# juanmc2005/diart

Hardware: AMD Instinct MI355X
Metric: real-time-factor xRT streams/GPU @500ms step (higher is better)
Workload: dtype f16x3

## Files before the change

### diart_amd/_lib.py

```python
from __future__ import annotations

import ctypes as C
import os
from pathlib import Path
from typing import Optional

EXPERIMENTS = os.environ.get("DZ_EXPERIMENTS", "0") not in ("", "0")
_LIB_PATH = Path(__file__).resolve().parent / ("libdiart_amd_exp.so" if EXPERIMENTS else "libdiart_amd.so")
_lib: Optional[C.CDLL] = None

c_float_p = C.POINTER(C.c_float)
c_double_p = C.POINTER(C.c_double)
c_int_p = C.POINTER(C.c_int)
vp = C.c_void_p


class SincNetWeights(C.Structure):
    _fields_ = [("wav_gamma", C.c_float), ("wav_beta", C.c_float)] + [
        (n, vp) for n in ("filt", "in0_g", "in0_b", "w1", "b1", "in1_g", "in1_b",
                          "w2", "b2", "in2_g", "in2_b", "w1_split", "w2_split", "filt_split")]


class SegWeights(C.Structure):
    _fields_ = [("sinc", SincNetWeights), ("wih", vp * 4), ("bih", vp * 4), ("whh", vp * 4),
# ... 89 lines not shown
    "dz_clu_step": (C.c_int, [vp, vp, C.c_int, C.c_int, vp, C.c_int, vp, vp]),
    "dz_clu_step_batch": (C.c_int, [C.POINTER(vp), C.c_int, vp, C.c_int, C.c_int, vp, C.c_int,
                                    vp, vp, C.c_int]),
    "dz_clu_get_centers": (C.c_int, [vp, vp, C.c_int]),
    "dz_clu_get_active": (C.c_int, [vp, vp]),
    "dz_clu_dim": (C.c_int, [vp]),
    "dz_clu_set_state": (C.c_int, [vp, vp, vp, C.c_int]),
    "dz_clu_destroy": (C.c_int, [vp]),
    "dz_lsap": (C.c_int, [vp, C.c_int, C.c_int, vp]),
    "dz_ring_create": (C.c_int, [vp, C.c_int, C.c_int, C.c_int, C.c_int, C.POINTER(vp)]),
    "dz_ring_reset": (C.c_int, [vp]),
    "dz_ring_destroy": (C.c_int, [vp]),
    "dz_ring_push": (C.c_int, [vp, vp, C.c_longlong, C.c_int, vp]),
    "dz_ring_window": (C.c_int, [vp, C.POINTER(vp), C.POINTER(C.c_longlong), C.POINTER(C.c_int)]),
    "dz_ring_read": (C.c_int, [vp, vp, vp]),
    "dz_ring_push_rows": (C.c_int, [vp, vp, C.c_longlong, C.c_int, C.POINTER(C.c_int), C.c_int, vp]),
    "dz_ring_filled_row": (C.c_int, [vp, C.c_int, C.POINTER(C.c_int)]),
    "dz_ring_gather": (C.c_int, [vp, C.POINTER(C.c_int), C.c_int, vp, C.c_longlong, vp]),
    "dz_ring_reset_row": (C.c_int, [vp, C.c_int]),
    "dz_tail_create": (C.c_int, [C.c_int, C.c_int, C.c_double, C.c_double, C.c_double, C.c_int,
                                 C.c_int, vp, C.POINTER(vp)]),
    "dz_tail_reset": (C.c_int, [vp]),
    "dz_tail_destroy": (C.c_int, [vp]),
    "dz_tail_max_rows": (C.c_int, [vp]),
    "dz_tail_step": (C.c_int, [vp, vp, C.c_double, C.c_double, vp, vp, vp, vp, vp, C.c_int, vp]),
    "dz_tail_step_batch": (C.c_int, [C.POINTER(vp), C.c_int, vp, vp, vp, vp, vp, vp, vp, vp,
                                     C.c_int, vp, C.c_int]),
    "dz_file_step_batch": (C.c_int, [C.POINTER(vp), C.POINTER(vp), C.c_int, vp, vp, vp, C.c_int, C.c_int, vp, C.c_int,
                                     C.c_int, vp, C.c_double, vp, C.c_int, vp, vp, C.c_int]),
    "dz_k_convgemm": (C.c_int, [vp, vp, vp]),
    "dz_k_gemm_f32": (C.c_int, [vp, vp, vp]),
    "dz_k_gemm_split": (C.c_int, [vp, vp, vp]),
    "dz_k_gemm_pre": (C.c_int, [vp, vp, vp]),
    "dz_k_mlp_head": (C.c_int, [vp, vp, C.c_longlong, vp, vp, vp, vp, vp, vp, C.c_int, C.c_int, C.c_int, C.c_int,
                                C.c_int, C.c_float, C.c_float, vp, vp, vp]),
    "dz_k_seg_head": (C.c_int, [vp, vp, vp, vp, C.c_int, C.c_int, C.c_int, C.c_int, C.c_int, vp, C.c_float,
                                C.c_float, C.c_int, vp, vp]),
    "dz_k_conv_pool": (C.c_int, [vp, vp, vp]),
    "dz_k_convgemm_ntile": (C.c_int, [C.c_int]),
    "dz_k_wave_stats": (C.c_int, [vp, vp, C.c_longlong, C.c_int, C.c_int, vp, vp]),
    "dz_k_sinc_conv0": (C.c_int, [vp, vp, C.c_longlong, C.c_int, C.c_int, vp, C.c_float,
                                  C.c_float, vp, vp, vp, vp]),
    "dz_k_sinc_conv0_split": (C.c_int, [vp, vp, C.c_longlong, C.c_int, C.c_int, vp, C.c_float,
                                        C.c_float, vp, vp, vp, vp]),
    "dz_k_conv0_split_ntile": (C.c_int, [C.c_int]),
    "dz_k_finalize_norm": (C.c_int, [vp, vp, C.c_int, C.c_int, C.c_int, C.c_int, vp, vp, vp, vp, vp]),
    "dz_k_lstm": (C.c_int, [vp, vp, vp, vp, C.c_int, C.c_int, vp]),
    "dz_k_lstm_mfma": (C.c_int, [vp, vp, vp, vp, C.c_int, C.c_int, C.c_int, C.c_int, vp]),
    "dz_k_lstm_planes": (C.c_int, [vp, vp, vp, vp, C.c_int, vp, C.c_longlong, C.c_int, C.c_int, vp]),
    "dz_k_stats_pool": (C.c_int, [vp, vp, C.c_int, C.c_int, C.c_int, vp, C.c_int, C.c_int,
                                  C.c_int, vp, C.c_int, vp]),
    "dz_k_powerset": (C.c_int, [vp, vp, C.c_int, C.c_int, C.c_int, vp, vp]),
}


EXPERIMENT_SIGNATURES = {
    "dz_k_gemm_g2": (C.c_int, [vp, vp, C.c_int, vp]),
    "dz_k_gemm_g3": (C.c_int, [vp, vp, C.c_int, vp]),
    "dz_k_conv_pool_debug": (C.c_int, [vp]),
    "dz_sinc_conv0_pair": (C.c_int, [vp, vp, vp, C.c_longlong, C.c_int, vp, vp, vp, vp]),
    "dz_k_sinc_conv0_pair": (C.c_int, [vp, vp, C.c_longlong, C.c_int, C.c_int, vp, vp, vp, C.c_float, C.c_float, vp, vp,
                                       vp, vp, vp]),
}


class ConvGemmDesc(C.Structure):
# ... 94 lines not shown
```

### diart_amd/csrc/api.hip

```cpp
#include "dz_common.h"

#include <stdarg.h>
#include <stdio.h>
#include <stdlib.h>
#include <string.h>
#include <mutex>
#include <new>

static thread_local char g_err[512] = "";
void dz_set_error(const char* fmt, ...) {
    va_list ap;
    va_start(ap, fmt);
    vsnprintf(g_err, sizeof(g_err), fmt, ap);
    va_end(ap);
}
extern "C" const char* dz_last_error(void) { return g_err; }
extern "C" int dz_version(void) { return DZ_VERSION; }
extern "C" int dz_abi_struct_sizes(int out[5]) {
    if (!out) return 2;
    out[0] = (int)sizeof(dz_sincnet_weights);
    out[1] = (int)sizeof(dz_seg_weights);
    out[2] = (int)sizeof(dz_emb_weights);
    out[3] = (int)sizeof(dz_ecapa_weights);
    out[4] = (int)sizeof(dz_convgemm_desc);
// ... 495 lines not shown
    const float* lin = nullptr;
    for (int layer = 0; layer < 4; ++layer) {
        DzConvGemm p;
        memset(&p, 0, sizeof(p));
        float* const gxl = layer == 0 ? s->gx0 : s->gx;
        p.W = s->w.wih[layer]; p.bias = s->w.bih[layer]; p.Y = gxl;
        p.taps = 1; p.dil = 1; p.Npad = 1024; p.Nstore = 1024; p.ldy = 1024; p.epi = DZ_EPI_BIAS;
        const bool do_proj = layer == 0 ? phase != 2 : phase != 1;
        const bool do_rec = phase != 1;
        if (layer == 0) {
            p.X = s->ss.y2;
            sinc_out_norm(p, s->w.sinc, s->g, s->ss, s->w.wih_split[0] != nullptr);
            p.B = B; p.Tin = p.Tout = p.Tstore = F; p.Cin = 64; p.K = 64; p.Kpad = 64; p.ldx = 64;
            p.xbs = (long long)F * 64; p.ybs = (long long)F * 1024;
        } else {
            p.X = lin;
            p.B = 1; p.Tin = p.Tout = p.Tstore = B * F; p.Cin = 256; p.K = 256; p.Kpad = 256;
            p.ldx = 256;
        }
        const bool pre0 = layer == 0 && s->pre && sinc_pre_split_ok(s->w.sinc, s->w.wih0_split_kb);
        if (layer == 0 && !pre0 && !s->w.wih_split[0] && sinc_f32_norm_pass(s->w.sinc)) {
            p.X = s->ss.y2s; p.norm_on_load = 0; p.npart = nullptr; p.nscale = p.nshift = nullptr;
            p.B = 1; p.Tin = p.Tout = p.Tstore = B * F; p.xbs = p.ybs = 0;
        }
        if (do_proj && pre0) {
            if ((rc = sinc_norm_split(s->w.sinc, s->g, s->ss, B, st))) return rc;
            p.X = nullptr; p.norm_on_load = 0; p.npart = nullptr; p.nscale = p.nshift = nullptr;
            p.B = 1; p.Tin = p.Tout = p.Tstore = B * F; p.xbs = p.ybs = 0;
        }
        if (do_proj)
        { ProfScope ps(layer == 0 ? T_PROJ0 : T_PROJ, B);
          if (pre0) {
              p.Xsplit = s->ss.y2s; p.xplane = rows * 64; p.Wsplit = s->w.wih0_split_kb;
              rc = dz_launch_gemm_pre(p, st);
          } else if (layer > 0 && s->pre) {
              p.X = nullptr; p.Xsplit = lin; p.xplane = rows * 256; p.Wsplit = s->w.wih_split[layer];
              rc = dz_launch_gemm_pre(p, st);
          } else {
              rc = run_gemm(p, s->w.wih_split[layer], st);
          }
          if (rc) return rc; }
        if (!do_rec) {
            s->front_B = B;
            return 0;
        }
        float* hout = (layer & 1) ? s->h1 : s->h0;
        { ProfScope ps(T_REC, B);
          float* hf = s->pre ? nullptr : hout;
          void* hs = s->pre ? (void*)hout : nullptr;
          rc = s->w.whh_split[layer]
                   ? dz_launch_lstm_mfma(gxl, s->w.whh_split[layer], hf, hs, rows * 256, B, F, 1,
                                         s->w.lstm_variant, st)
                   : dz_launch_lstm(gxl, s->w.whh[layer], hf, hs, rows * 256, B, F, 1, st);
          if (rc) return rc; }
        if (layer == 0) {
            DZ_HIP(hipEventRecord(s->ev_gx0_free, st));
            s->front_B = 0;
        }
        lin = hout;
    }
    DzConvGemm p;
    memset(&p, 0, sizeof(p));
    p.B = 1; p.Tin = p.Tout = p.Tstore = B * F; p.taps = 1; p.dil = 1;
    p.W = s->w.lin0_w; p.bias = s->w.lin0_b;
    p.Cin = 256; p.K = 256; p.Kpad = 256; p.ldx = 256; p.Npad = 128; p.Nstore = 128; p.ldy = 128;
    p.epi = DZ_EPI_BIAS_LEAKY;
    if (s->pre && mlp_head_enabled() && !(d_osp && normalize) && s->w.num_classes <= 8) {
        DzMlpHead m{};
        m.Xsplit = lin; m.xplane = rows * 256;
        m.W0split = s->w.lin0_split; m.W1split = s->w.lin1_split;
// ... 349 lines not shown
                               int n_streams, int k_local, int g_global, int dim, double* d_out,
                               void* stream) {
    DZ_REQUIRE(ctx && d_emb && d_centers && d_out, "dz_cdist_cosine: NULL argument");
    DZ_REQUIRE(n_streams >= 1 && k_local >= 1 && g_global >= 1 && dim >= 1,
               "dz_cdist_cosine: empty input");
    DZ_HIP(hipSetDevice(ctx->device));
    return dz_launch_cdist(d_emb, d_centers, n_streams, k_local, g_global, dim, d_out,
                           (hipStream_t)stream);
}

extern "C" int dz_k_convgemm(dz_ctx* ctx, const dz_convgemm_desc* d, void* stream) {
    DZ_REQUIRE(ctx && d, "dz_k_convgemm: NULL argument");
    DZ_HIP(hipSetDevice(ctx->device));
    DzRangeScope range_scope(ctx->oflag_dev);
    return dz_launch_convgemm(*d, (hipStream_t)stream);
}
extern "C" int dz_k_gemm_f32(dz_ctx* ctx, const dz_convgemm_desc* d, void* stream) {
    DZ_REQUIRE(ctx && d, "dz_k_gemm_f32: NULL argument");
    DZ_HIP(hipSetDevice(ctx->device));
    return dz_launch_gemm_f32(*d, (hipStream_t)stream);
}
extern "C" int dz_k_gemm_split(dz_ctx* ctx, const dz_convgemm_desc* d, void* stream) {
    DZ_REQUIRE(ctx && d, "dz_k_gemm_split: NULL argument");
    DZ_HIP(hipSetDevice(ctx->device));
    DzRangeScope range_scope(ctx->oflag_dev);
    return dz_launch_gemm_split(*d, (hipStream_t)stream);
}
extern "C" int dz_k_gemm_pre(dz_ctx* ctx, const dz_convgemm_desc* d, void* stream) {
    DZ_REQUIRE(ctx && d, "dz_k_gemm_pre: NULL argument");
    DZ_HIP(hipSetDevice(ctx->device));
    DzRangeScope range_scope(ctx->oflag_dev);
    return dz_launch_gemm_pre(*d, (hipStream_t)stream);
}
#ifdef DZ_EXPERIMENTS
extern "C" int dz_k_gemm_g2(dz_ctx* ctx, const dz_convgemm_desc* d, int row_fragments, void* stream) {
    DZ_REQUIRE(ctx && d, "dz_k_gemm_g2: NULL argument");
    DZ_REQUIRE(d->Wsplit && d->Xsplit && (d->Y || d->Ysplit) && d->B == 1 && d->K == d->Kpad && d->K == d->taps * d->Cin &&
                   d->Cin % 32 == 0 && d->Npad % 128 == 0 && d->pad == 0 && !d->X2 && !d->rowbias && d->ksplit <= 1 &&
                   !d->norm_on_load && d->Tout > 0 && d->Tout == d->Tin - (d->taps - 1) * d->dil && d->ldx % 32 == 0 &&
                   d->xplane % d->ldx == 0 && d->xplane / d->ldx >= d->Tin,
               "dz_k_gemm_g2: the requirements of dz_k_gemm_pre apply");
    DZ_HIP(hipSetDevice(ctx->device));
    DzRangeScope range_scope(ctx->oflag_dev);
    DzConvGemm p = *d;
    if (!p.oflag) p.oflag = ctx->oflag_dev;
    return dz_launch_gemm_g2(p, row_fragments, (hipStream_t)stream);
}
extern "C" int dz_k_gemm_g3(dz_ctx* ctx, const dz_convgemm_desc* d, int row_fragments, void* stream) {
    DZ_REQUIRE(ctx && d, "dz_k_gemm_g3: NULL argument");
    DZ_REQUIRE(d->Wsplit && d->Xsplit && (d->Y || d->Ysplit) && d->B == 1 && d->K == d->Kpad && d->K == d->taps * d->Cin &&
                   d->Cin % 32 == 0 && d->Npad % 128 == 0 && d->pad == 0 && !d->X2 && !d->rowbias && d->ksplit <= 1 &&
                   !d->norm_on_load && d->Tout > 0 && d->Tout == d->Tin - (d->taps - 1) * d->dil && d->ldx % 32 == 0 &&
                   d->xplane % d->ldx == 0 && d->xplane / d->ldx >= d->Tin,
               "dz_k_gemm_g3: the requirements of dz_k_gemm_pre apply");
    DZ_HIP(hipSetDevice(ctx->device));
    DzRangeScope range_scope(ctx->oflag_dev);
    DzConvGemm p = *d;
    if (!p.oflag) p.oflag = ctx->oflag_dev;
    return dz_launch_gemm_g3(p, row_fragments, (hipStream_t)stream);
}
#endif
extern "C" int dz_k_mlp_head(dz_ctx* ctx, const void* xsplit, long long xplane, const void* w0split,
                             const void* w1split, const float* b0, const float* b1, const float* cw,
                             const float* cb, int rows, int frames, int classes, int speakers, int powerset,
                             float gamma, float beta, float* d_seg, float* d_weights, void* stream) {
    DZ_REQUIRE(ctx, "dz_k_mlp_head: NULL argument");
// ... 161 lines not shown
```

### diart_amd/csrc/dz_common.h

```cpp
#pragma once
#include <hip/hip_runtime.h>
#include <hip/hip_ext.h>
#include <stdint.h>
#include <stddef.h>
#include <mutex>
#include "../../include/diart_amd.h"

#ifdef DZ_EXPERIMENTS
#include <stdlib.h>
static inline const char* dz_exp_env(const char* name) { return getenv(name); }
#else
#define dz_exp_env(name) ((const char*)nullptr)
#endif
enum { DZ_OPT_F32_GEMM = 0, DZ_OPT_POOL_FUSE, DZ_OPT_PACK_CACHE, DZ_OPT_COUNT };
int dz_option(int id);

typedef float f32x4 __attribute__((ext_vector_type(4)));
typedef float f32x2 __attribute__((ext_vector_type(2)));

#define DZ_MFMA(a, b, c) __builtin_amdgcn_mfma_f32_16x16x4f32((a), (b), (c), 0, 0, 0)

#define DZ_LEAKY_SLOPE 0.01f

struct DzAttrOnce {
// ... 166 lines not shown
                         hipStream_t st);
int dz_launch_wave_stats_combine(const float* mom, int B, int S, float* stats, hipStream_t st);
int dz_launch_sinc_conv0(const float* wave, long long stride, int B, int S, const float* stats,
                         int stats_are_moments, float gamma, float beta, const float* filt,
                         float* y0, int P0, float* partials, int ntile, hipStream_t st);
int dz_launch_sinc_conv0_split(const float* wave, long long stride, int B, int S, const float* stats,
                               int stats_are_moments, float gamma, float beta, const void* filt_split,
                               float* y0, int P0, float* partials, int ntile, hipStream_t st, const void* ffrag = nullptr);
int dz_sinc_bank_frag_bytes();
int dz_launch_sinc_bank_frag(const void* fsp, void* frag, hipStream_t st);
int dz_conv0_split_ntile(int F0);
int dz_launch_sinc_conv0_pair(const float* wave, long long stride, int B, int S, const float* moments,
                              const void* pair_planes, const float* pair_bsum, float gamma_seg, float gamma_emb,
                              float* y0_seg, float* y0_emb, int P0, float* part_seg, float* part_emb, int ntile,
                              hipStream_t st);
int dz_launch_finalize_norm(const float* partials, int B, int ntile, int C, int T,
                            const float* gamma, const float* beta, float* scale, float* shift,
                            hipStream_t st);

typedef dz_convgemm_desc DzConvGemm;
constexpr int DZ_EPI_TG = 0x100;
int dz_launch_convgemm(const DzConvGemm& p, hipStream_t st);
bool dz_gemm_f32_ok(const DzConvGemm& p);
int dz_launch_gemm_f32(const DzConvGemm& p, hipStream_t st);
int dz_launch_gemm_split(const DzConvGemm& p, hipStream_t st);
int dz_launch_norm_f32(const float* y, const float* part, int ntile, int P, const float* gamma, const float* beta,
                       float* out, int B, hipStream_t st);
int dz_launch_norm_split(const float* y, const float* part, int ntile, int P, const float* gamma, const float* beta,
                         void* planes, long long plane, int B, hipStream_t st);
int dz_launch_conv_pool(const DzConvGemm& p, hipStream_t st, const void* wfrag = nullptr);
int dz_conv_pool_wfrag_bytes(int Cin);
int dz_launch_conv_pool_wfrag(int Cin, const void* wsplit, int Kpad, void* out, hipStream_t st);
int dz_launch_gemm_pre(const DzConvGemm& p, hipStream_t st);
#ifdef DZ_EXPERIMENTS
int dz_launch_gemm_g2(const DzConvGemm& p, int mt, hipStream_t st);
int dz_g2_default_mt();
#endif
int dz_gemm_gen();
#ifdef DZ_EXPERIMENTS
int dz_launch_gemm_g3(const DzConvGemm& p, int mt, hipStream_t st);
int dz_g3_error(int reset);
#endif
__device__ __forceinline__ float dz_pool_weight(const float* wr, int Fw, int T, int t) {
    const int F = Fw < 0 ? -Fw : Fw;
    if (F == T) return wr[t];
    const float scale = (float)F / (float)T;
    if (Fw < 0) {
        int i = (int)floorf((float)t * scale);
        if (i > F - 1) i = F - 1;
        return wr[i];
    }
    float src = scale * ((float)t + 0.5f) - 0.5f;
    if (src < 0.f) src = 0.f;
    const int i0 = (int)src;
    const int i1 = i0 + (i0 < F - 1 ? 1 : 0);
    const float l1 = src - (float)i0;
    return (1.f - l1) * wr[i0] + l1 * wr[i1];
}

struct DzPoolFuse {
    const float* w;
    int Fw, K;
    int P, T;
    int np;
    float* part;
    float* s0;
// ... 147 lines not shown
```

### diart_amd/csrc/k_gemm_pre.hip

```cpp
#include "dz_common.h"
#include <stdlib.h>
#include <type_traits>

namespace {

typedef _Float16 f16x8 __attribute__((ext_vector_type(8)));
typedef _Float16 f16x2 __attribute__((ext_vector_type(2)));
typedef float f32x16 __attribute__((ext_vector_type(16)));

constexpr int BM = 128, BN = 128, KT = 32;
constexpr int PLANE_B = 128 * 64;
constexpr int plane_a(int MW) { return 64 * MW * 64; }
constexpr int stage_bytes(int MW) { return 2 * plane_a(MW) + 2 * PLANE_B; }
constexpr size_t lds_bytes(int MW) { return 2 * (size_t)stage_bytes(MW) + 3 * BN * sizeof(float); }
constexpr int MW_BIG = 6;
constexpr float LO_UNSCALE = 1.f / 2048.f;

__device__ __forceinline__ float leaky(float v) { return fmaxf(v, v * DZ_LEAKY_SLOPE); }

constexpr int YT_PITCH = 132;
constexpr int POOL_PAR = BM * YT_PITCH * 4;
constexpr int POOL_WT = POOL_PAR + 3 * BN * 4;
constexpr int POOL_RED = POOL_WT + 4 * BM * 4;
constexpr int POOL_S0 = POOL_RED + 2 * 2 * 4 * BN * 4;
constexpr size_t POOL_LDS = POOL_S0 + 8 * 8 * 2 * 4 + 8 * 2 * 4;

template <int EPI, int MW, int MT, int NT, bool ILV = false, bool POOL = false>
__device__ __forceinline__ void gemm_pre_tile(const DzConvGemm& p, const int t0, const int n0, char* smem,
                                              const int flags = 0, const DzPoolFuse* q = nullptr) {
    constexpr int PLANE_A = plane_a(MW), STAGE = stage_bytes(MW), PAR_OFF = POOL ? POOL_PAR : 2 * STAGE;
    static_assert(!POOL || (MW == 2 && MT == 2 && NT == 2), "pooled epilogue: 128 x 128 tiles only");
    const int tid = threadIdx.x;
    const int w = __builtin_amdgcn_readfirstlane(tid >> 6), l = tid & 63;

// ... 437 lines not shown
            for (int k = 0; k < KK; ++k)
                *reinterpret_cast<f32x2*>(red + (wv_ * 4 + k) * BN + c2) = (f32x2){S[k][0], S[k][1]};
            __syncthreads();
            const int b = b0 + part;
            if (wv_ == 0 && b < nx) {
                const int piece = t0 / BM - (b * P) / BM;
#pragma unroll
                for (int k = 0; k < KK; ++k) {
                    f32x2 m2 = {0.f, 0.f};
#pragma unroll
                    for (int v = 0; v < 4; ++v) m2 += *reinterpret_cast<const f32x2*>(red + (v * 4 + k) * BN + c2);
                    float* o = q->part + ((((long long)b * q->np + piece) * K + k) * p.Npad + n0 + c2) * 2;
                    *reinterpret_cast<f32x4*>(o) = (f32x4){mean[k][0], m2[0], mean[k][1], m2[1]};
                    if (n0 == 0 && c2 == 0) {
                        float* so = q->s0 + (((long long)b * q->np + piece) * K + k) * 2;
                        so[0] = s0f[(part * 4 + k) * 2];
                        so[1] = s0f[(part * 4 + k) * 2 + 1];
                    }
                }
            }
        };
        for (int part = 0; part < (rb < BM ? 2 : 1); ++part) {
            if (part) __syncthreads();
            switch (K) {
                case 1: pool_part(std::integral_constant<int, 1>{}, part); break;
                case 2: pool_part(std::integral_constant<int, 2>{}, part); break;
                case 3: pool_part(std::integral_constant<int, 3>{}, part); break;
                default: pool_part(std::integral_constant<int, 4>{}, part); break;
            }
        }
    }
}

template <int EPI, bool ILV>
__global__ __launch_bounds__(256, 2) void gemm_pre_kernel(DzConvGemm p, int mbig, int msmall, int flags) {
    extern __shared__ __attribute__((aligned(16))) char smem[];
#ifndef DZ_EXPERIMENTS
    flags = 0;
#endif
    const int gy = p.Npad / BN, L = blockIdx.x;
    if (L < mbig * gy) {
        int bx, by, bz;
        dz_tile_map_lin(L, mbig, gy, 1, p.agroup, bx, by, bz);
        gemm_pre_tile<EPI, 2, 2, 2, ILV>(p, bx * BM, by * BN, smem, flags);
    } else {
        const int Ls = L - mbig * gy, gys = 2 * gy;
        const int xcd = Ls & 7, j = Ls >> 3;
        const int ms = (j / gys) * 8 + xcd, by = j % gys;
        if (ms >= msmall) return;
        gemm_pre_tile<EPI, 2, 1, 1>(p, mbig * BM + ms * 64, by * 64, smem);
    }
}

__global__ __launch_bounds__(256, 2) void gemm_pre_pool_kernel(DzConvGemm p, DzPoolFuse q, int gx, int flags) {
    extern __shared__ __attribute__((aligned(16))) char smem[];
    const int gy = p.Npad / BN;
    int bx, by, bz;
    dz_tile_map_lin(blockIdx.x, gx, gy, 1, p.agroup, bx, by, bz);
#ifndef DZ_EXPERIMENTS
    flags = 0;
#endif
    gemm_pre_tile<DZ_EPI_TDNN, 2, 2, 2, true, true>(p, bx * BM, by * BN, smem, flags, &q);
}

template <int EPI>
__global__ __launch_bounds__(64 * 2 * MW_BIG) void gemm_pre_big_kernel(DzConvGemm p) {
    extern __shared__ __attribute__((aligned(16))) char smem[];
    const int gy = p.Npad / BN, gx = (p.Tout + 64 * MW_BIG - 1) / (64 * MW_BIG);
    int bx, by, bz;
// ... 13 lines not shown
        const char* e = dz_exp_env("DZ_GP_LOOP");
        return !(e && e[0] == '0');
    }();
    return on;
}

int dbg_flags() {
    static const int f = [] {
        const char* e = dz_exp_env("DZ_GP_DBG");
        return e ? atoi(e) : 0;
    }();
    return f;
}

bool tail_tiles_enabled() {
    static const bool on = [] {
        const char* e = dz_exp_env("DZ_GEMM_TAIL");
        return e && e[0] == '1';
    }();
    return on;
}
int wg_slots() {
    static const int slots = [] {
        int dev = 0, cus = 256;
        if (hipGetDevice(&dev) == hipSuccess) hipDeviceGetAttribute(&cus, hipDeviceAttributeMultiprocessorCount, dev);
        return 2 * (cus > 0 ? cus : 256);
    }();
    return slots;
}

template <int EPI>
int launch(const DzConvGemm& p, hipStream_t st) {
    static DzAttrOnce attr_ilv;
    DZ_HIP(attr_ilv.raise((const void*)gemm_pre_kernel<EPI, true>, (int)lds_bytes(2)));
    const int gx = (p.Tout + BM - 1) / BM, gy = p.Npad / BN, slots = wg_slots();
#ifdef DZ_EXPERIMENTS
    static DzAttrOnce attr_once, attr_big;
    DZ_HIP(attr_once.raise((const void*)gemm_pre_kernel<EPI, false>, (int)lds_bytes(2)));
    {
        const int gxb = (p.Tout + 64 * MW_BIG - 1) / (64 * MW_BIG);
        const int mode = big_tiles_mode();
        if (mode == 1 && gxb >= 8) {
            DZ_HIP(attr_big.raise((const void*)gemm_pre_big_kernel<EPI>, (int)lds_bytes(MW_BIG)));
            DZ_LAUNCH((gemm_pre_big_kernel<EPI>), dim3(gxb * gy), dim3(64 * 2 * MW_BIG), lds_bytes(MW_BIG), st, p);
            DZ_HIP(hipGetLastError());
            return 0;
        }
    }
#endif
    int mbig = gx;
    const int tiles = gx * gy, rem = tiles % slots;
    if (4 * tiles < slots)
        mbig = 0;
    else if (tail_tiles_enabled() && rem != 0 && 4 * rem < 3 * slots)
        mbig = (tiles / slots) * slots / gy;
    const int rows_left = p.Tout - mbig * BM;
    const int msmall = rows_left > 0 ? (rows_left + 63) / 64 : 0;
    const int nwg = mbig * gy + ((msmall + 7) / 8) * 8 * (2 * gy);
#ifdef DZ_EXPERIMENTS
    if (!interleaved_loop())
        DZ_LAUNCH((gemm_pre_kernel<EPI, false>), dim3(nwg), dim3(256), lds_bytes(2), st, p, mbig, msmall, 0);
    else
#endif
        DZ_LAUNCH((gemm_pre_kernel<EPI, true>), dim3(nwg), dim3(256), lds_bytes(2), st, p, mbig, msmall, dbg_flags());
    DZ_HIP(hipGetLastError());
    return 0;
}

}

int dz_gemm_gen() {
    static const int gen = [] {
        const char* e = dz_exp_env("DZ_GEMM_GEN");
        const int v = e ? atoi(e) : 1;
        return v == 2 || v == 3 ? v : 1;
    }();
    return gen;
}

bool dz_gemm_pre_pool_ok(const DzConvGemm& p) {
    const int gx = (p.Tout + BM - 1) / BM, gy = p.Npad / BN;
    return 4 * gx * gy >= wg_slots();
}

int dz_launch_gemm_pre_pool(const DzConvGemm& p_in, const DzPoolFuse& q, hipStream_t st) {
    DzConvGemm p = p_in;
    if (!p.oflag) p.oflag = dz_cur_oflag;
    DZ_REQUIRE(p.Wsplit && p.Xsplit && q.part && q.s0, "gemm_pre_pool: NULL operand");
    DZ_REQUIRE(p.epi == DZ_EPI_TDNN && p.B == 1 && p.taps == 1 && p.K == p.Kpad && p.Cin % KT == 0 &&
                   p.Npad % BN == 0 && p.Tout == p.Tin,
               "gemm_pre_pool: built for the flattened 1 x 1 TDNN layer");
    DZ_REQUIRE(q.np == dz_pool_pieces(q.P), "gemm_pre_pool: np must be dz_pool_pieces(P)");
    DZ_REQUIRE(q.K >= 1 && q.K <= 4 && q.P >= BM && q.T >= 2 && q.T <= q.P && p.Tout % q.P == 0 && (q.Fw >= 2 || q.Fw <= -2),
               "gemm_pre_pool: 1..4 speakers, chunk pitch >= 128 rows (got K %d, P %d, T %d)", q.K, q.P, q.T);
    DZ_REQUIRE(p.ldx > 0 && p.ldx % KT == 0 && p.xplane % p.ldx == 0 && p.xplane / p.ldx >= p.Tin,
               "gemm_pre_pool: kb-major input planes need ldx %% 32 == 0 and xplane = rows * ldx with rows >= Tin");
    DZ_REQUIRE(p.xplane * 2 < (1ll << 31) && (long long)p.Npad * p.Kpad * 2 < (1ll << 31),
               "gemm_pre_pool: operand plane exceeds the 2 GiB buffer-offset range");
    static const int pool_ag = [] {
        const char* e = dz_exp_env("DZ_POOL_AG");
        return e && atoi(e) > 0 ? atoi(e) : 1;
    }();
    if (!p.agroup) p.agroup = pool_ag;
    static DzAttrOnce attr_once;
    DZ_HIP(attr_once.raise((const void*)gemm_pre_pool_kernel, (int)POOL_LDS));
    const int gx = (p.Tout + BM - 1) / BM, gy = p.Npad / BN;
    DZ_LAUNCH(gemm_pre_pool_kernel, dim3(gx * gy), dim3(256), POOL_LDS, st, p, q, gx, dbg_flags());
    DZ_HIP(hipGetLastError());
    return 0;
}

int dz_launch_gemm_pre(const DzConvGemm& p_in, hipStream_t st) {
    DzConvGemm p = p_in;
    if (!p.oflag) p.oflag = dz_cur_oflag;
    DZ_REQUIRE(p.Wsplit != nullptr && p.Xsplit != nullptr,
               "gemm_pre: Wsplit / Xsplit (f16 hi/lo planes of W and of the input) are NULL");
    DZ_REQUIRE(p.Y != nullptr || p.Ysplit != nullptr, "gemm_pre: no output");
    DZ_REQUIRE(p.B == 1, "gemm_pre: flattened layers only (B = 1)");
    DZ_REQUIRE(p.K == p.Kpad && p.K == p.taps * p.Cin && p.Cin % KT == 0,
               "gemm_pre: K = taps * Cin without padding, Cin a multiple of 32");
    DZ_REQUIRE(p.Npad % BN == 0, "gemm_pre: Npad must be a multiple of 128");
    DZ_REQUIRE(p.Tout > 0 && p.Tout == p.Tin - (p.taps - 1) * p.dil, "gemm_pre: Tout mismatch");
    DZ_REQUIRE(p.pad == 0 && p.X2 == nullptr && p.rowbias == nullptr && p.ksplit <= 1 && !p.norm_on_load,
               "gemm_pre: padding / second input / row bias / split-K / norm-on-load are not built here");
    DZ_REQUIRE(p.ldx > 0 && p.ldx % KT == 0 && p.xplane % p.ldx == 0 && p.xplane / p.ldx >= p.Tin,
               "gemm_pre: kb-major input planes need ldx %% 32 == 0 and xplane = rows * ldx with rows >= Tin");
    DZ_REQUIRE(p.xplane * 2 < (1ll << 31) && (long long)p.Npad * p.Kpad * 2 < (1ll << 31),
               "gemm_pre: operand plane exceeds the 2 GiB buffer-offset range");
    DZ_REQUIRE(p.Ysplit == nullptr || (p.ldy > 0 && p.ldy % KT == 0 && p.yplane % p.ldy == 0 && p.yplane / p.ldy >= p.Tout &&
                                       p.Npad <= p.ldy && p.yplane * 2 < (1ll << 31)),
               "gemm_pre: kb-major output planes need ldy %% 32 == 0, yplane = rows * ldy with rows >= Tout, Npad <= ldy");
    DZ_REQUIRE(p.Y == nullptr || (p.ldy % 4 == 0 && ((uintptr_t)p.Y & 15) == 0),
               "gemm_pre: f32 output needs ldy a multiple of 4 and a 16-byte aligned base");
#ifdef DZ_EXPERIMENTS
    if (dz_gemm_gen() >= 2 && 4 * ((p.Tout + BM - 1) / BM) * (p.Npad / BN) >= wg_slots()) {
        static const int g3_min_k = [] {
            const char* e = dz_exp_env("DZ_G3_MINK");
            return e ? atoi(e) : 1024;
        }();
        if (dz_gemm_gen() == 3) {
            if (p.K >= g3_min_k) return dz_launch_gemm_g3(p, 0, st);
        } else {
            return dz_launch_gemm_g2(p, 0, st);
        }
    }
#endif
    switch (p.epi) {
        case DZ_EPI_BIAS: return launch<DZ_EPI_BIAS>(p, st);
        case DZ_EPI_BIAS_LEAKY: return launch<DZ_EPI_BIAS_LEAKY>(p, st);
        case DZ_EPI_TDNN: return launch<DZ_EPI_TDNN>(p, st);
        case DZ_EPI_RELU_BN: return launch<DZ_EPI_RELU_BN>(p, st);
    }
    dz_set_error("gemm_pre: epilogue %d is not built on the pre-split path", p.epi);
    return 2;
}
```

### include/diart_amd.h

```cpp
#ifndef DIART_AMD_H
#define DIART_AMD_H

#ifdef __cplusplus
extern "C" {
#endif

#define DZ_VERSION 230

typedef struct dz_ctx dz_ctx;
typedef struct dz_seg dz_seg;
typedef struct dz_emb dz_emb;
typedef struct dz_clu dz_clu;

const char* dz_last_error(void);
int dz_version(void);
int dz_set_option(const char* name, int value);
int dz_get_option(const char* name, int* value);
int dz_has_experiments(void);
int dz_host_pool_set_spin(int microseconds);

int dz_ctx_create(int hip_device, dz_ctx** out);
int dz_ctx_destroy(dz_ctx* ctx);
int dz_range_check(dz_ctx* ctx, int reset);

// ... 166 lines not shown
    const float* bias;
    const float* e0;
    const float* e1;
    const float* nscale;
    const float* nshift;
    float* Y;
    float* partials;
    int B, Tin, Tout, Cin, taps, dil, K, Kpad, Npad, Nstore, ldx, ldy, nld, Tstore;
    long long xbs, ybs;
    int norm_on_load;
    int epi;
    int ksplit;
    long long ysplit;
    int agroup;
    int pad;
    const float* X2;
    const float* rowbias;
    const void* Wsplit;
    const void* Xsplit;
    long long xplane;
    void* Ysplit;
    long long yplane;
    const float* npart;
    const float* ngamma;
    const float* nbeta;
    int npart_tiles, npart_T;
    int* oflag;
    const int* Tdev;
} dz_convgemm_desc;
int dz_k_convgemm(dz_ctx* ctx, const dz_convgemm_desc* desc, void* stream);
int dz_k_gemm_f32(dz_ctx* ctx, const dz_convgemm_desc* desc, void* stream);
int dz_k_gemm_split(dz_ctx* ctx, const dz_convgemm_desc* desc, void* stream);
int dz_k_gemm_pre(dz_ctx* ctx, const dz_convgemm_desc* desc, void* stream);
int dz_k_mlp_head(dz_ctx* ctx, const void* xsplit, long long xplane, const void* w0split, const void* w1split,
                  const float* b0, const float* b1, const float* cw, const float* cb, int rows, int frames,
                  int classes, int speakers, int powerset, float gamma, float beta, float* d_seg,
                  float* d_weights, void* stream);
int dz_k_seg_head(dz_ctx* ctx, const float* m1, const float* cw, const float* cb, int batch, int frames,
                  int classes, int speakers, int powerset, float* d_seg, float gamma, float beta,
                  int normalize, float* d_weights, void* stream);
int dz_k_conv_pool(dz_ctx* ctx, const dz_convgemm_desc* desc, void* stream);
int dz_k_convgemm_ntile(int t_out);
int dz_k_wave_stats(dz_ctx* ctx, const float* d_wave, long long stride, int batch, int samples,
                    float* d_stats, void* stream);
int dz_k_sinc_conv0(dz_ctx* ctx, const float* d_wave, long long stride, int batch, int samples,
                    const float* d_stats, float gamma, float beta, const float* d_filt,
                    float* d_y0, float* d_partials, void* stream);
int dz_k_sinc_conv0_split(dz_ctx* ctx, const float* d_wave, long long stride, int batch, int samples,
                          const float* d_stats, float gamma, float beta, const void* d_filt_split,
                          float* d_y0, float* d_partials, void* stream);
int dz_k_conv0_split_ntile(int samples);
int dz_k_finalize_norm(dz_ctx* ctx, const float* d_partials, int batch, int ntile, int channels,
                       int frames, const float* d_gamma, const float* d_beta, float* d_scale,
                       float* d_shift, void* stream);
int dz_k_lstm(dz_ctx* ctx, const float* d_gx, const float* d_whh, float* d_hout, int batch,
              int frames, void* stream);
int dz_k_lstm_mfma(dz_ctx* ctx, const float* d_gx, const void* d_whh_split, float* d_hout,
                   int batch, int frames, int unit_major, int variant, void* stream);
int dz_k_lstm_planes(dz_ctx* ctx, const float* d_gx, const float* d_whh, const void* d_whh_split,
                     int variant, void* d_hsplit, long long hplane, int batch, int frames, void* stream);
int dz_k_stats_pool(dz_ctx* ctx, const float* d_x, int frames, int channels, int ldx,
                    const float* d_weights, int weight_frames, int rows, int rows_per_x,
                    float* d_out, int ldo, void* stream);
int dz_k_powerset(dz_ctx* ctx, const float* d_logits, int rows, int classes, int speakers,
                  float* d_out, void* stream);

// ... 65 lines not shown
```

Baseline: 33140.

## Add persistent pipelined GEMM path for LSTM input projections

Adds a specialised persistent-tile path inside the pre-split GEMM kernel for the LSTM input projections (bias epilogue, K 64/256, N 1024). Each workgroup loops over tiles and prefetches the next tile's operands into LDS via buffer-to-LDS loads while finishing the current one. Bias is staged in LDS, and MFMA issue is hand-interleaved with loads under sched barriers. The goal is to cut launch-tail and prologue cost for large tile counts, at the price of hardcoded vmcnt waits and narrow shape constraints. Small problems still fall back to the old launch.

```diff
diff --git a/diart_amd/_lib.py b/diart_amd/_lib.py
--- a/diart_amd/_lib.py
+++ b/diart_amd/_lib.py
@@ -145,6 +145,7 @@
     "dz_k_gemm_f32": (C.c_int, [vp, vp, vp]),
     "dz_k_gemm_split": (C.c_int, [vp, vp, vp]),
     "dz_k_gemm_pre": (C.c_int, [vp, vp, vp]),
+    "dz_k_gemm_proj": (C.c_int, [vp, vp, vp]),
     "dz_k_mlp_head": (C.c_int, [vp, vp, C.c_longlong, vp, vp, vp, vp, vp, vp, C.c_int, C.c_int, C.c_int, C.c_int,
                                 C.c_int, C.c_float, C.c_float, vp, vp, vp]),
     "dz_k_seg_head": (C.c_int, [vp, vp, vp, vp, C.c_int, C.c_int, C.c_int, C.c_int, C.c_int, vp, C.c_float,
diff --git a/diart_amd/csrc/api.hip b/diart_amd/csrc/api.hip
--- a/diart_amd/csrc/api.hip
+++ b/diart_amd/csrc/api.hip
@@ -551,10 +551,10 @@
         { ProfScope ps(layer == 0 ? T_PROJ0 : T_PROJ, B);
           if (pre0) {
               p.Xsplit = s->ss.y2s; p.xplane = rows * 64; p.Wsplit = s->w.wih0_split_kb;
-              rc = dz_launch_gemm_pre(p, st);
+              rc = dz_launch_gemm_proj(p, st);
           } else if (layer > 0 && s->pre) {
               p.X = nullptr; p.Xsplit = lin; p.xplane = rows * 256; p.Wsplit = s->w.wih_split[layer];
-              rc = dz_launch_gemm_pre(p, st);
+              rc = dz_launch_gemm_proj(p, st);
           } else {
               rc = run_gemm(p, s->w.wih_split[layer], st);
           }
@@ -970,6 +970,12 @@
     DzRangeScope range_scope(ctx->oflag_dev);
     return dz_launch_gemm_pre(*d, (hipStream_t)stream);
 }
+extern "C" int dz_k_gemm_proj(dz_ctx* ctx, const dz_convgemm_desc* d, void* stream) {
+    DZ_REQUIRE(ctx && d, "dz_k_gemm_proj: NULL argument");
+    DZ_HIP(hipSetDevice(ctx->device));
+    DzRangeScope range_scope(ctx->oflag_dev);
+    return dz_launch_gemm_proj(*d, (hipStream_t)stream);
+}
 #ifdef DZ_EXPERIMENTS
 extern "C" int dz_k_gemm_g2(dz_ctx* ctx, const dz_convgemm_desc* d, int row_fragments, void* stream) {
     DZ_REQUIRE(ctx && d, "dz_k_gemm_g2: NULL argument");
diff --git a/diart_amd/csrc/dz_common.h b/diart_amd/csrc/dz_common.h
--- a/diart_amd/csrc/dz_common.h
+++ b/diart_amd/csrc/dz_common.h
@@ -222,6 +222,7 @@
 int dz_conv_pool_wfrag_bytes(int Cin);
 int dz_launch_conv_pool_wfrag(int Cin, const void* wsplit, int Kpad, void* out, hipStream_t st);
 int dz_launch_gemm_pre(const DzConvGemm& p, hipStream_t st);
+int dz_launch_gemm_proj(const DzConvGemm& p, hipStream_t st);
 #ifdef DZ_EXPERIMENTS
 int dz_launch_gemm_g2(const DzConvGemm& p, int mt, hipStream_t st);
 int dz_g2_default_mt();
diff --git a/diart_amd/csrc/k_gemm_pre.hip b/diart_amd/csrc/k_gemm_pre.hip
--- a/diart_amd/csrc/k_gemm_pre.hip
+++ b/diart_amd/csrc/k_gemm_pre.hip
@@ -1,5 +1,6 @@
 #include "dz_common.h"
 #include <stdlib.h>
+#include <algorithm>
 #include <type_traits>
 
 namespace {
@@ -503,9 +504,214 @@
     }
 }
 
+constexpr int PROJ_NPC = 8;
+constexpr int PROJ_NST = 16;
+constexpr size_t PROJ_LDS = 2 * (size_t)stage_bytes(2) + 1024 * sizeof(float);
+
+template <int EPI>
+__device__ __forceinline__ void gemm_proj_tiles(const DzConvGemm& p, char* smem, const int ntiles) {
+    constexpr int PLANE_A = plane_a(2), STAGE = stage_bytes(2);
+    const int tid = threadIdx.x;
+    const int w = __builtin_amdgcn_readfirstlane(tid >> 6), l = tid & 63;
+    const int gx = (p.Tout + BM - 1) / BM, gy = p.Npad / BN, G = gridDim.x;
+    int L = blockIdx.x;
+    if (L >= ntiles) return;
+    const bool isB = w >= 2;
+    const int r2 = w & 1;
+    const unsigned short* src = isB ? reinterpret_cast<const unsigned short*>(p.Wsplit)
+                                    : reinterpret_cast<const unsigned short*>(p.Xsplit);
+    const int prows = isB ? p.Npad : (int)((unsigned)p.xplane / (unsigned)p.ldx);
+    const long long plane_el = isB ? (long long)p.Npad * p.Kpad : p.xplane;
+    const unsigned nbytes = (unsigned)((long long)prows * (isB ? p.Kpad : p.ldx) * 2);
+    const __amdgpu_buffer_rsrc_t rs_hi = __builtin_amdgcn_make_buffer_rsrc((void*)src, 0, nbytes, 0x00020000);
+    const __amdgpu_buffer_rsrc_t rs_lo = __builtin_amdgcn_make_buffer_rsrc((void*)(src + plane_el), 0, nbytes, 0x00020000);
+    constexpr int vstep = 16 * 64;
+    const int lane_off = (l >> 2) * 64 + (((l & 3) ^ ((l >> 4) & 3)) << 4) + r2 * vstep;
+    const int kb_bytes = prows * 64;
+    char* const dbase = smem + (isB ? 2 * PLANE_A : 0) + r2 * 1024;
+    const int dplane = isB ? PLANE_B : PLANE_A;
+    auto tile_of = [&](const int Lt, int& t0, int& n0) __attribute__((always_inline)) {
+        int bx, by, bz;
+        dz_tile_map_lin(Lt, gx, gy, 1, p.agroup, bx, by, bz);
+        t0 = bx * BM;
+        n0 = by * BN;
+    };
+    int vofs_n = 0, soff_n = 0, stage_n = 0;
+    auto piece = [&](int j) __attribute__((always_inline)) {
+        __builtin_amdgcn_raw_ptr_buffer_load_lds(j >= 4 ? rs_lo : rs_hi,
+            (__attribute__((address_space(3))) void*)(dbase + stage_n * STAGE + (j >= 4) * dplane + (j & 3) * 2048), 16,
+            vofs_n + (j & 3) * 2 * vstep, soff_n, 0, 0);
+    };
+
+    float* const par = reinterpret_cast<float*>(smem + 2 * STAGE);
+    for (int c = 4 * tid; c < p.Npad; c += 4 * 256)
+        *reinterpret_cast<f32x4*>(par + c) = *reinterpret_cast<const f32x4*>(p.bias + c);
+
+    int t0, n0;
+    tile_of(L, t0, n0);
+    int vofs = (isB ? n0 : t0) * 64 + lane_off;
+    vofs_n = vofs;
+#pragma unroll
+    for (int kt = 0; kt < 2; ++kt) {
+        soff_n = kt * kb_bytes;
+        stage_n = kt;
+#pragma unroll
+        for (int j = 0; j < PROJ_NPC; ++j) piece(j);
+    }
+
+    const int li = l & 31, g = l >> 5;
+    const int wm = w >> 1, wn = w & 1;
+    const int sw = (li >> 2) & 3;
+    int foff[2];
+#pragma unroll
+    for (int ks = 0; ks < 2; ++ks) foff[ks] = li * 64 + (((2 * ks + g) ^ sw) << 4);
+    const char* sa0 = smem + (wm * 64) * 64;
+    const char* sb0 = smem + 2 * PLANE_A + (wn * 64) * 64;
+    const int nk = p.Kpad / KT;
+    const unsigned nrec = __builtin_amdgcn_readfirstlane((unsigned)(4ll * p.Tout * p.ldy));
+    const __amdgpu_buffer_rsrc_t ry = __builtin_amdgcn_make_buffer_rsrc((void*)p.Y, 0, nrec, 0x00020000);
+    bool first = true;
+    f32x16 accm[2][2], accx[2][2];
+
+#define DZ_RD(base, plane, t, ks) (*reinterpret_cast<const f16x8*>((base) + (plane) + (t) * 2048 + foff[ks]))
+#define DZ_MM(mt, nt)                                                                                     \
+    accx[mt][nt] = __builtin_amdgcn_mfma_f32_32x32x16_f16(bh[nt], al[mt], accx[mt][nt], 0, 0, 0);          \
+    accm[mt][nt] = __builtin_amdgcn_mfma_f32_32x32x16_f16(bh[nt], ah[mt], accm[mt][nt], 0, 0, 0);          \
+    accx[mt][nt] = __builtin_amdgcn_mfma_f32_32x32x16_f16(bl[nt], ah[mt], accx[mt][nt], 0, 0, 0)
+#define DZ_PIN() __builtin_amdgcn_sched_barrier(0)
+    auto body = [&](const int kt, auto more_c) __attribute__((always_inline)) {
+        constexpr bool more = decltype(more_c)::value;
+        const char* sa = sa0 + (kt & 1) * STAGE;
+        const char* sb = sb0 + (kt & 1) * STAGE;
+        f16x8 ah[2], al[2], bh[2], bl[2];
+        bh[0] = DZ_RD(sb, 0, 0, 0); al[0] = DZ_RD(sa, PLANE_A, 0, 0); ah[0] = DZ_RD(sa, 0, 0, 0);
+        bl[0] = DZ_RD(sb, PLANE_B, 0, 0);
+        bh[1] = DZ_RD(sb, 0, 1, 0); bl[1] = DZ_RD(sb, PLANE_B, 1, 0);
+        ah[1] = DZ_RD(sa, 0, 1, 0); al[1] = DZ_RD(sa, PLANE_A, 1, 0);
+        DZ_PIN();
+        accx[0][0] = __builtin_amdgcn_mfma_f32_32x32x16_f16(bh[0], al[0], accx[0][0], 0, 0, 0);
+        accm[0][0] = __builtin_amdgcn_mfma_f32_32x32x16_f16(bh[0], ah[0], accm[0][0], 0, 0, 0);
+        DZ_PIN();
+        if (more) piece(0);
+        DZ_PIN();
+        accx[0][0] = __builtin_amdgcn_mfma_f32_32x32x16_f16(bl[0], ah[0], accx[0][0], 0, 0, 0);
+        accx[0][1] = __builtin_amdgcn_mfma_f32_32x32x16_f16(bh[1], al[0], accx[0][1], 0, 0, 0);
+        DZ_PIN();
+        if (more) piece(1);
+        DZ_PIN();
+        accm[0][1] = __builtin_amdgcn_mfma_f32_32x32x16_f16(bh[1], ah[0], accm[0][1], 0, 0, 0);
+        accx[0][1] = __builtin_amdgcn_mfma_f32_32x32x16_f16(bl[1], ah[0], accx[0][1], 0, 0, 0);
+        DZ_PIN();
+        if (more) piece(2);
+        ah[0] = DZ_RD(sa, 0, 0, 1); al[0] = DZ_RD(sa, PLANE_A, 0, 1);
+        DZ_PIN();
+        accx[1][1] = __builtin_amdgcn_mfma_f32_32x32x16_f16(bh[1], al[1], accx[1][1], 0, 0, 0);
+        accm[1][1] = __builtin_amdgcn_mfma_f32_32x32x16_f16(bh[1], ah[1], accm[1][1], 0, 0, 0);
+        DZ_PIN();
+        if (more) piece(3);
+        DZ_PIN();
+        accx[1][1] = __builtin_amdgcn_mfma_f32_32x32x16_f16(bl[1], ah[1], accx[1][1], 0, 0, 0);
+        accx[1][0] = __builtin_amdgcn_mfma_f32_32x32x16_f16(bh[0], al[1], accx[1][0], 0, 0, 0);
+        DZ_PIN();
+        if (more) piece(4);
+        bh[1] = DZ_RD(sb, 0, 1, 1); bl[1] = DZ_RD(sb, PLANE_B, 1, 1);
+        DZ_PIN();
+        accm[1][0] = __builtin_amdgcn_mfma_f32_32x32x16_f16(bh[0], ah[1], accm[1][0], 0, 0, 0);
+        accx[1][0] = __builtin_amdgcn_mfma_f32_32x32x16_f16(bl[0], ah[1], accx[1][0], 0, 0, 0);
+        DZ_PIN();
+        if (more) piece(5);
+        bh[0] = DZ_RD(sb, 0, 0, 1); bl[0] = DZ_RD(sb, PLANE_B, 0, 1);
+        ah[1] = DZ_RD(sa, 0, 1, 1); al[1] = DZ_RD(sa, PLANE_A, 1, 1);
+        DZ_PIN();
+        accx[0][1] = __builtin_amdgcn_mfma_f32_32x32x16_f16(bh[1], al[0], accx[0][1], 0, 0, 0);
+        accm[0][1] = __builtin_amdgcn_mfma_f32_32x32x16_f16(bh[1], ah[0], accm[0][1], 0, 0, 0);
+        DZ_PIN();
+        if (more) piece(6);
+        DZ_PIN();
+        accx[0][1] = __builtin_amdgcn_mfma_f32_32x32x16_f16(bl[1], ah[0], accx[0][1], 0, 0, 0);
+        accx[0][0] = __builtin_amdgcn_mfma_f32_32x32x16_f16(bh[0], al[0], accx[0][0], 0, 0, 0);
+        DZ_PIN();
+        if (more) piece(7);
+        DZ_PIN();
+        accm[0][0] = __builtin_amdgcn_mfma_f32_32x32x16_f16(bh[0], ah[0], accm[0][0], 0, 0, 0);
+        accx[0][0] = __builtin_amdgcn_mfma_f32_32x32x16_f16(bl[0], ah[0], accx[0][0], 0, 0, 0);
+        DZ_MM(1, 0);
+        DZ_MM(1, 1);
+    };
+
+    for (;;) {
+        const int Ln = L + G;
+        const bool has_next = Ln < ntiles;
+        int t0n = 0, n0n = 0;
+        if (has_next) tile_of(Ln, t0n, n0n);
+#pragma unroll
+        for (int mt = 0; mt < 2; ++mt)
+#pragma unroll
+            for (int nt = 0; nt < 2; ++nt)
+#pragma unroll
+                for (int r = 0; r < 16; ++r) accm[mt][nt][r] = accx[mt][nt][r] = 0.f;
+        static_assert(PROJ_NPC == 8 && PROJ_NST == 16, "the vmcnt immediates below");
+        if (first) asm volatile("s_waitcnt vmcnt(8) lgkmcnt(0)\n\ts_barrier" ::: "memory");
+        else asm volatile("s_waitcnt vmcnt(24) lgkmcnt(0)\n\ts_barrier" ::: "memory");
+        body(0, std::false_type{});
+        for (int kt = 1; kt < nk; ++kt) {
+            if (kt == 1 && !first) asm volatile("s_waitcnt vmcnt(16) lgkmcnt(0)\n\ts_barrier" ::: "memory");
+            else asm volatile("s_waitcnt vmcnt(0) lgkmcnt(0)\n\ts_barrier" ::: "memory");
+            const bool last = kt + 1 == nk;
+            vofs_n = last && has_next ? (isB ? n0n : t0n) * 64 + lane_off : vofs;
+            soff_n = last ? 0 : (kt + 1) * kb_bytes;
+            stage_n = (kt + 1) & 1;
+            body(kt, std::true_type{});
+        }
+        if (has_next) {
+            asm volatile("s_waitcnt lgkmcnt(0)\n\ts_barrier" ::: "memory");
+            soff_n = kb_bytes; stage_n = 1;
+#pragma unroll
+            for (int j = 0; j < PROJ_NPC; ++j) piece(j);
+        }
+        const float* parl = par + n0 + wn * 64 + 4 * g;
+#pragma unroll
+        for (int mt = 0; mt < 2; ++mt) {
+            const int t = t0 + wm * 64 + mt * 32 + li;
+            const int vo = t < p.Tout ? (t * p.ldy + 4 * g) * 4 : (int)0x80000000;
+#pragma unroll
+            for (int nt = 0; nt < 2; ++nt) {
+                const int cb = n0 + wn * 64 + nt * 32;
+                const int so = __builtin_amdgcn_readfirstlane(cb * 4);
+#pragma unroll
+                for (int k = 0; k < 4; ++k) {
+                    asm volatile("" ::: "memory");
+                    const f32x4 bv = *reinterpret_cast<const f32x4*>(parl + nt * 32 + 8 * k);
+                    f32x4 v;
+#pragma unroll
+                    for (int e = 0; e < 4; ++e) {
+                        v[e] = (accm[mt][nt][4 * k + e] + accx[mt][nt][4 * k + e] * LO_UNSCALE) + bv[e];
+                    }
+                    typedef unsigned u32x4 __attribute__((ext_vector_type(4)));
+                    __builtin_amdgcn_raw_buffer_store_b128(__builtin_bit_cast(u32x4, v), ry, vo + 32 * k, so, 0);
+                }
+            }
+        }
+        if (!has_next) break;
+        L = Ln; t0 = t0n; n0 = n0n;
+        vofs = (isB ? n0 : t0) * 64 + lane_off;
+        first = false;
+    }
+    asm volatile("s_waitcnt vmcnt(0)" ::: "memory");
+#undef DZ_RD
+#undef DZ_MM
+#undef DZ_PIN
+}
+
 template <int EPI, bool ILV>
-__global__ __launch_bounds__(256, 2) void gemm_pre_kernel(DzConvGemm p, int mbig, int msmall, int flags) {
+__global__ __launch_bounds__(256, 2) void gemm_pre_kernel(DzConvGemm p, int mbig, int msmall, int flags, int ptiles) {
     extern __shared__ __attribute__((aligned(16))) char smem[];
+    if constexpr (EPI == DZ_EPI_BIAS && ILV) {
+        if (ptiles > 0) {
+            gemm_proj_tiles<EPI>(p, smem, ptiles);
+            return;
+        }
+    }
 #ifndef DZ_EXPERIMENTS
     flags = 0;
 #endif
@@ -585,7 +791,7 @@
 template <int EPI>
 int launch(const DzConvGemm& p, hipStream_t st) {
     static DzAttrOnce attr_ilv;
-    DZ_HIP(attr_ilv.raise((const void*)gemm_pre_kernel<EPI, true>, (int)lds_bytes(2)));
+    DZ_HIP(attr_ilv.raise((const void*)gemm_pre_kernel<EPI, true>, (int)std::max(lds_bytes(2), PROJ_LDS)));
     const int gx = (p.Tout + BM - 1) / BM, gy = p.Npad / BN, slots = wg_slots();
 #ifdef DZ_EXPERIMENTS
     static DzAttrOnce attr_once, attr_big;
@@ -612,10 +818,10 @@
     const int nwg = mbig * gy + ((msmall + 7) / 8) * 8 * (2 * gy);
 #ifdef DZ_EXPERIMENTS
     if (!interleaved_loop())
-        DZ_LAUNCH((gemm_pre_kernel<EPI, false>), dim3(nwg), dim3(256), lds_bytes(2), st, p, mbig, msmall, 0);
+        DZ_LAUNCH((gemm_pre_kernel<EPI, false>), dim3(nwg), dim3(256), lds_bytes(2), st, p, mbig, msmall, 0, 0);
     else
 #endif
-        DZ_LAUNCH((gemm_pre_kernel<EPI, true>), dim3(nwg), dim3(256), lds_bytes(2), st, p, mbig, msmall, dbg_flags());
+        DZ_LAUNCH((gemm_pre_kernel<EPI, true>), dim3(nwg), dim3(256), lds_bytes(2), st, p, mbig, msmall, dbg_flags(), 0);
     DZ_HIP(hipGetLastError());
     return 0;
 }
@@ -663,9 +869,8 @@
     return 0;
 }
 
-int dz_launch_gemm_pre(const DzConvGemm& p_in, hipStream_t st) {
-    DzConvGemm p = p_in;
-    if (!p.oflag) p.oflag = dz_cur_oflag;
+namespace {
+int check_pre(const DzConvGemm& p) {
     DZ_REQUIRE(p.Wsplit != nullptr && p.Xsplit != nullptr,
                "gemm_pre: Wsplit / Xsplit (f16 hi/lo planes of W and of the input) are NULL");
     DZ_REQUIRE(p.Y != nullptr || p.Ysplit != nullptr, "gemm_pre: no output");
@@ -685,6 +890,14 @@
                "gemm_pre: kb-major output planes need ldy %% 32 == 0, yplane = rows * ldy with rows >= Tout, Npad <= ldy");
     DZ_REQUIRE(p.Y == nullptr || (p.ldy % 4 == 0 && ((uintptr_t)p.Y & 15) == 0),
                "gemm_pre: f32 output needs ldy a multiple of 4 and a 16-byte aligned base");
+    return 0;
+}
+}
+
+int dz_launch_gemm_pre(const DzConvGemm& p_in, hipStream_t st) {
+    DzConvGemm p = p_in;
+    if (!p.oflag) p.oflag = dz_cur_oflag;
+    if (int rc = check_pre(p)) return rc;
 #ifdef DZ_EXPERIMENTS
     if (dz_gemm_gen() >= 2 && 4 * ((p.Tout + BM - 1) / BM) * (p.Npad / BN) >= wg_slots()) {
         static const int g3_min_k = [] {
@@ -707,3 +920,20 @@
     dz_set_error("gemm_pre: epilogue %d is not built on the pre-split path", p.epi);
     return 2;
 }
+
+int dz_launch_gemm_proj(const DzConvGemm& p_in, hipStream_t st) {
+    DzConvGemm p = p_in;
+    if (!p.oflag) p.oflag = dz_cur_oflag;
+    if (int rc = check_pre(p)) return rc;
+    DZ_REQUIRE(p.epi == DZ_EPI_BIAS && p.taps == 1 && (p.Kpad == 64 || p.Kpad == 256) && p.Npad == 1024 &&
+                   p.Nstore == p.Npad && p.Y != nullptr && p.Ysplit == nullptr && 4ll * p.Tout * p.ldy < (1ll << 31),
+               "gemm_proj: built for the LSTM input projections (bias epilogue, K 64 or 256, N 1024, f32 output "
+               "below 2 GiB; got epi %d, taps %d, Kpad %d, Npad %d, Nstore %d)", p.epi, p.taps, p.Kpad, p.Npad, p.Nstore);
+    const int tiles = ((p.Tout + BM - 1) / BM) * (p.Npad / BN), slots = wg_slots();
+    if (tiles < slots) return launch<DZ_EPI_BIAS>(p, st);
+    static DzAttrOnce attr_proj;
+    DZ_HIP(attr_proj.raise((const void*)gemm_pre_kernel<DZ_EPI_BIAS, true>, (int)std::max(lds_bytes(2), PROJ_LDS)));
+    DZ_LAUNCH((gemm_pre_kernel<DZ_EPI_BIAS, true>), dim3(slots & ~7), dim3(256), PROJ_LDS, st, p, 0, 0, 0, tiles);
+    DZ_HIP(hipGetLastError());
+    return 0;
+}
diff --git a/include/diart_amd.h b/include/diart_amd.h
--- a/include/diart_amd.h
+++ b/include/diart_amd.h
@@ -222,6 +222,7 @@
 int dz_k_gemm_f32(dz_ctx* ctx, const dz_convgemm_desc* desc, void* stream);
 int dz_k_gemm_split(dz_ctx* ctx, const dz_convgemm_desc* desc, void* stream);
 int dz_k_gemm_pre(dz_ctx* ctx, const dz_convgemm_desc* desc, void* stream);
+int dz_k_gemm_proj(dz_ctx* ctx, const dz_convgemm_desc* desc, void* stream);
 int dz_k_mlp_head(dz_ctx* ctx, const void* xsplit, long long xplane, const void* w0split, const void* w1split,
                   const float* b0, const float* b1, const float* cw, const float* cb, int rows, int frames,
                   int classes, int speakers, int powerset, float gamma, float beta, float* d_seg,
```

Result: no change. 32940, median of 6 (-0.6%).
